# eniac/flamingo

Hardware: AMD Instinct MI355X
Metric: device-resident aggregate+unmask GB/s, N clients × L int32 per round (higher is better)
Workload: dtype u32

## Files before the change

### flamingo_amd/_lib.py

```python
from __future__ import annotations

import ctypes
import os

HERE = os.path.dirname(os.path.abspath(__file__))
LIB_PATH = os.environ.get("FLM_LIB_PATH") or os.path.join(HERE, "lib", "libflamingo_hip.so")

_u8p = ctypes.POINTER(ctypes.c_uint8)
_i8p = ctypes.POINTER(ctypes.c_int8)
_u32p = ctypes.POINTER(ctypes.c_uint32)
_i64p = ctypes.POINTER(ctypes.c_int64)
_f32p = ctypes.POINTER(ctypes.c_float)
_vp = ctypes.c_void_p
_sz = ctypes.c_size_t
_u64 = ctypes.c_uint64
_int = ctypes.c_int

SIGNATURES = {
    "flm_device_count": (_int, []),
    "flm_init": (_int, [ctypes.POINTER(_vp), _int]),
    "flm_free": (None, [_vp]),
    "flm_last_error": (ctypes.c_char_p, [_vp]),
    "flm_version": (ctypes.c_char_p, []),
    "flm_ctx_stream": (_vp, [_vp]),
# ... 32 lines not shown
    "flm_last_plan": (_int, [_vp, ctypes.POINTER(_int), ctypes.POINTER(_int), ctypes.POINTER(_int),
                             ctypes.POINTER(_int)]),
    "flm_set_tuning": (_int, [_vp, ctypes.c_char_p, _int]),
    "flm_get_tuning": (_int, [_vp, ctypes.c_char_p, ctypes.POINTER(_int)]),
    "flm_plan_aggregate": (_int, [_int, _int, _sz, _int, _int, _sz, _sz, _sz, _u64, _vp, _int,
                                  ctypes.POINTER(_int), ctypes.POINTER(_int)]),
    "flm_ec_combine": (_int, [_vp, _u8p, _u8p, _u8p, _int, _int, _int, _u8p, _u8p, _u32p]),
    "flm_ec_combine_dev": (_int, [_vp, _vp, _vp, _vp, _int, _int, _int, _vp, _vp, _vp, _vp]),
    "flm_ec_mul": (_int, [_vp, _u8p, _u8p, _int, _u8p, _u32p]),
    "flm_hash_to_curve": (_int, [_vp, _u8p, _u32p, _int, _u8p, _u32p]),
    "flm_hash_to_curve_decimal": (_int, [_vp, ctypes.c_uint32, _int, _u8p, _u32p]),
    "flm_hash_to_curve_decimal_dev": (_int, [_vp, ctypes.c_uint32, _int, _vp, _vp, _vp]),
    "flm_shamir_combine": (_int, [_vp, _u8p, _u8p, _int, _int, _u8p]),
    "flm_shamir_combine_dev": (_int, [_vp, _vp, _vp, _int, _int, _vp, _vp]),
    "flm_shamir_deal": (_int, [_vp, _u8p, _int, _int, _u32p, _int, _u8p]),
    "flm_shamir_deal_dev": (_int, [_vp, _vp, _int, _int, _vp, _int, _vp, _vp]),
    "flm_aes_gcm_xor": (_int, [_vp, _u8p, _u8p, _int, _u8p, _u8p, _sz, _int]),
    "flm_aes_gcm_xor_dev": (_int, [_vp, _vp, _vp, _int, _vp, _vp, _sz, _int, _vp]),
    "flm_aes_gcm_seal": (_int, [_vp, _u8p, _u8p, _int, _u8p, _sz, _u8p, _u8p, _sz, _u8p, _int]),
    "flm_aes_gcm_seal_dev": (_int, [_vp, _vp, _vp, _int, _vp, _sz, _vp, _vp, _sz, _vp, _int, _vp]),
    "flm_aes_gcm_open": (_int, [_vp, _u8p, _u8p, _int, _u8p, _sz, _u8p, _u8p, _u8p, _sz, _u8p, _int]),
    "flm_aes_gcm_open_dev": (_int, [_vp, _vp, _vp, _int, _vp, _sz, _vp, _vp, _vp, _sz, _vp, _int, _vp]),
    "flm_ecdsa_verify": (_int, [_vp, _u8p, _u8p, _u8p, _int, _u8p, _u32p]),
    "flm_ecdsa_verify_dev": (_int, [_vp, _vp, _vp, _vp, _int, _vp, _vp, _vp]),
    "flm_feldman_verify": (_int, [_vp, _u8p, _int, _int, _u32p, _u32p, _int, _u8p, _int, _u8p, _u8p, _u32p]),
    "flm_feldman_verify_dev": (_int, [_vp, _vp, _int, _int, _vp, _vp, _int, _vp, _int, _vp, _vp, _vp, _vp]),
    "flm_pair_units_dev": (_int, [_vp, _vp, _vp, _int, _vp, _vp, _vp, _sz, _vp, _int, _int, _vp]),
    "flm_flag_set_dev": (_int, [_vp, _vp, _vp]),
    "flm_cu_count": (_int, [_vp, _vp]),
    "flm_stream_create_cu_mask": (_int, [_vp, _vp, _int, _vp]),
    "flm_stream_destroy": (_int, [_vp, _vp]),
    "flm_shard_bounds": (_int, [_sz, _int, _int, ctypes.POINTER(_sz), ctypes.POINTER(_sz), ctypes.POINTER(_sz)]),
    "flm_client_bounds": (_int, [_int, _int, _int, ctypes.POINTER(_int), ctypes.POINTER(_int)]),
    "flm_rccl_available": (_int, []),
    "flm_comm_unique_id": (_int, [_vp]),
    "flm_comm_init_rank": (_int, [_vp, _int, _int, _vp]),
    "flm_comm_size": (_int, [_vp, ctypes.POINTER(_int), ctypes.POINTER(_int)]),
    "flm_comm_destroy": (_int, [_vp]),
    "flm_reduce_scatter_dev": (_int, [_vp, _vp, _vp, _sz, _vp]),
    "flm_all_gather_dev": (_int, [_vp, _vp, _vp, _sz, _vp]),
    "flm_group_init": (_int, [ctypes.POINTER(_vp), _int, ctypes.POINTER(_int)]),
    "flm_group_free": (None, [_vp]),
    "flm_group_last_error": (ctypes.c_char_p, [_vp]),
    "flm_group_size": (_int, [_vp]),
    "flm_group_is_loopback": (_int, [_vp]),
    "flm_group_init_flags": (_int, [ctypes.POINTER(_vp), _int, ctypes.POINTER(_int), ctypes.c_uint]),
    "flm_group_has_rccl": (_int, [_vp]),
    "flm_group_ctx": (_vp, [_vp, _int]),
    "flm_group_sync": (_int, [_vp]),
    "flm_group_aggregate_unmask": (_int, [_vp, ctypes.POINTER(_u32p), _int, _u8p, _i8p, _int, _sz, _u32p]),
    "flm_group_aggregate_unmask_dev": (_int, [_vp, ctypes.POINTER(_vp), _sz, ctypes.POINTER(_int),
                                              ctypes.POINTER(_vp), ctypes.POINTER(_vp), _int, _sz,
                                              ctypes.POINTER(_vp)]),
    "flm_store_create": (_int, [ctypes.POINTER(_vp), _vp, _vp, _sz, _int]),
    "flm_store_free": (None, [_vp]),
    "flm_store_last_error": (ctypes.c_char_p, [_vp]),
    "flm_store_count": (_int, [_vp]),
    "flm_store_add": (_int, [_vp, ctypes.c_int64, _vp, _sz]),
    "flm_store_partial": (_int, [_vp]),
    "flm_store_partial_wait": (_int, [_vp, ctypes.POINTER(ctypes.c_float)]),
    "flm_store_partial_host": (_int, [_vp, _u32p]),
    "flm_store_unmask": (_int, [_vp, _u8p, _i8p, _int, _u32p]),
    "flm_store_unmask_f32": (_int, [_vp, _u8p, _i8p, _int, _int, ctypes.c_int64, _f32p]),
    "flm_store_unmask_unpack_f32": (_int, [_vp, _u8p, _i8p, _int, _sz, _int, ctypes.c_float, _int, ctypes.c_int64, _f32p]),
    "flm_store_unmask_unpack_noise_f32": (_int, [_vp, _u8p, _i8p, _int, _sz, _int, ctypes.c_float, _int, _int,
                                                 ctypes.c_int64, _f32p]),
# ... 49 lines not shown
```

### flamingo_amd/csrc/flm_comm.hip

```cpp
#include <hip/hip_runtime.h>
#include <rccl/rccl.h>

#include <dlfcn.h>

#include <algorithm>
#include <cstdarg>
#include <cstdio>
#include <cstdlib>
#include <cstring>
#include <mutex>
#include <string>
#include <thread>
#include <vector>

#include "../../include/flamingo_hip.h"
#include "flm_internal.h"

namespace {

struct Rccl {
    void *h = nullptr;
    std::string err;
    ncclResult_t (*GetUniqueId)(ncclUniqueId *) = nullptr;
    ncclResult_t (*CommInitRank)(ncclComm_t *, int, ncclUniqueId, int) = nullptr;
// ... 119 lines not shown
        if (!c) continue;
        (void)hipSetDevice(flm::rt::device_of(ctxs[q]));
        if (c->comm && r) (void)r->CommDestroy(c->comm);
        delete c;
        *flm::rt::comm_slot(ctxs[q]) = nullptr;
    }
}
}

namespace {
constexpr uint64_t kShardAlign = 1024;

uint64_t padded_len(uint64_t L, int G) {
    const uint64_t q = kShardAlign * (uint64_t)G;
    return (L + q - 1) / q * q;
}
}

extern "C" {

int flm_shard_bounds(size_t L, int n_ranks, int rank, size_t *lo, size_t *hi, size_t *shard_words) {
    if (n_ranks < 1 || rank < 0 || rank >= n_ranks || !lo || !hi) return FLM_EINVAL;
    const uint64_t S = padded_len(L, n_ranks) / n_ranks;
    *lo = (size_t)std::min<uint64_t>((uint64_t)rank * S, L);
    *hi = (size_t)std::min<uint64_t>((uint64_t)(rank + 1) * S, L);
    if (shard_words) *shard_words = (size_t)S;
    return 0;
}

int flm_client_bounds(int N, int n_ranks, int rank, int *c0, int *c1) {
    if (N < 0 || n_ranks < 1 || rank < 0 || rank >= n_ranks || !c0 || !c1) return FLM_EINVAL;
    *c0 = (int)((int64_t)N * rank / n_ranks);
    *c1 = (int)((int64_t)N * (rank + 1) / n_ranks);
    return 0;
}

int flm_rccl_available(void) {
    Rccl *r = rccl();
    if (!r) {
        flm::rt::set_error(nullptr, FLM_EHIP, rccl_state().err.c_str());
        return 0;
    }
    return 1;
}

int flm_comm_unique_id(uint8_t id_out[128]) {
    static_assert(sizeof(ncclUniqueId) == 128, "ncclUniqueId must be 128 bytes");
    if (!id_out) return FLM_EINVAL;
    Rccl *r = rccl();
    if (!r) return flm::rt::set_error(nullptr, FLM_EHIP, "RCCL unavailable");
    ncclUniqueId id;
    ncclResult_t e = r->GetUniqueId(&id);
    if (e != ncclSuccess) return flm::rt::set_error(nullptr, FLM_EHIP, r->GetErrorString(e));
    std::memcpy(id_out, &id, sizeof id);
    return 0;
}

int flm_comm_init_rank(flm_ctx *ctx, int n_ranks, int rank, const uint8_t id[128]) {
    if (!ctx) return flm::rt::set_error(nullptr, FLM_EINVAL, "ctx is NULL");
    if (n_ranks < 1 || rank < 0 || rank >= n_ranks || !id) return fail_ctx(ctx, FLM_EINVAL, "bad rank %d of %d", rank, n_ranks);
    Rccl *r = rccl();
    if (!r) return rccl_missing(ctx);
    flm::comm_release(ctx);
    flm::rt::DeviceScope dev_scope_;
    FLM_HIPC(ctx, dev_scope_.set(flm::rt::device_of(ctx)));
    ncclUniqueId uid;
// ... 54 lines not shown

}

struct flm_group {
    int n = 0;
    std::vector<int> dev;
    std::vector<flm_ctx *> ctx;
    bool loopback = false;
    bool clique = false;
    struct Rank {
        uint32_t *partial = nullptr, *shard = nullptr;
        size_t cap_partial = 0, cap_shard = 0;
        hipEvent_t done = nullptr;
        hipEvent_t xdone = nullptr;
        bool xpending = false;
        size_t dirty = 0;
    };
    std::vector<Rank> rk;
    uint32_t *hout = nullptr;
    size_t hout_cap = 0;
    std::string err;
};

namespace {

int gfail(flm_group *g, int code, const std::string &msg) {
    if (g) g->err = msg;
    flm::rt::set_error(nullptr, code, msg.c_str());
    return code;
}

bool sharded(const flm_group *g) { return g->n > 1 || g->clique; }

int grow(flm_group *g, int r, uint32_t *&p, size_t &cap, size_t words) {
    if (words <= cap) return 0;
    (void)hipSetDevice(g->dev[r]);
    if (p) (void)hipFree(p);
    p = nullptr;
    cap = 0;
    hipError_t e = hipMalloc(&p, std::max<size_t>(words, 64) * sizeof(uint32_t));
    if (e == hipSuccess)
        e = hipMemsetAsync(p, 0, std::max<size_t>(words, 64) * sizeof(uint32_t), flm::rt::stream_of(g->ctx[r]));
    if (e != hipSuccess) return gfail(g, FLM_ENOMEM, std::string("group buffer: ") + hipGetErrorString(e));
    cap = words;
    return 0;
}

int rank_error(flm_group *g, int r, int rc) {
    return gfail(g, rc, "rank " + std::to_string(r) + ": " + flm_last_error(g->ctx[r]));
}

int exchange(flm_group *g, uint64_t S, const std::vector<uint32_t *> &shards) {
    const int G = g->n;
    if (g->loopback) {
        std::vector<const uint32_t *> parts(G);
        for (int r = 0; r < G; ++r) parts[r] = g->rk[r].partial;
        for (int r = 0; r < G; ++r) {
            hipStream_t s = flm::rt::stream_of(g->ctx[r]);
            for (int q = 0; q < G; ++q)
                if (q != r && hipStreamWaitEvent(s, g->rk[q].done, 0) != hipSuccess)
                    return gfail(g, FLM_EHIP, "hipStreamWaitEvent");
            hipError_t e = flm::launch_shard_sum(parts.data(), G, (uint64_t)r * S, S, shards[r], s);
            if (e != hipSuccess) return gfail(g, FLM_EHIP, std::string("shard_sum: ") + hipGetErrorString(e));
            if (hipEventRecord(g->rk[r].xdone, s) != hipSuccess) return gfail(g, FLM_EHIP, "hipEventRecord");
            g->rk[r].xpending = true;
        }
// ... 144 lines not shown
    return 0;
}

int flm_group_aggregate_unmask(flm_group *g, const uint32_t *const *rows, int N, const uint8_t *seeds,
                               const int8_t *signs, int K, size_t L, uint32_t *out) {
    flm::rt::DeviceScope dev_scope_;
    if (!g) return gfail(nullptr, FLM_EINVAL, "group is NULL");
    if (N < 0 || K < 0) return gfail(g, FLM_EINVAL, "negative N or K");
    if (L == 0) return 0;
    if (!out || (N > 0 && !rows) || (K > 0 && (!seeds || !signs))) return gfail(g, FLM_EINVAL, "NULL argument");
    int rc_ = 0;
    const int G = g->n;
    const bool X = sharded(g);
    const uint64_t Lp = padded_len(L, G), S = Lp / G;
    for (int r = 0; r < G; ++r) {
        if (X && (rc_ = grow(g, r, g->rk[r].partial, g->rk[r].cap_partial, Lp))) return rc_;
        if ((rc_ = grow(g, r, g->rk[r].shard, g->rk[r].cap_shard, S))) return rc_;
    }
    for (int r = 0; r < G; ++r)
        if ((rc_ = wait_previous_exchange(g, r))) return rc_;
    for (int r = 0; X && r < G; ++r)
        if ((rc_ = clear_stale_tail(g, r, L))) return rc_;
    if (g->hout_cap < L) {
        if (g->hout) (void)hipHostFree(g->hout);
        g->hout = nullptr;
        g->hout_cap = 0;
        if (hipHostMalloc(&g->hout, L * sizeof(uint32_t), hipHostMallocPortable) != hipSuccess)
            return gfail(g, FLM_ENOMEM, "group: pinned output buffer");
        g->hout_cap = L;
    }
    std::vector<int> rcs(G, 0);
    auto work = [&](int r) {
        int c0, c1;
        size_t lo, hi;
        flm_client_bounds(N, G, r, &c0, &c1);
        flm_shard_bounds(L, G, r, &lo, &hi, nullptr);
        rcs[r] = flm::rt::host_round_async(g->ctx[r], rows ? rows + c0 : nullptr, c1 - c0, seeds, signs, K, L, lo, hi,
                                           X ? g->rk[r].partial : g->rk[r].shard);
        if (!rcs[r] && hipEventRecord(g->rk[r].done, flm::rt::stream_of(g->ctx[r])) != hipSuccess) rcs[r] = FLM_EHIP;
    };
    if (G == 1) {
        work(0);
    } else {
        std::vector<std::thread> th;
        for (int r = 0; r < G; ++r) th.emplace_back(work, r);
        for (auto &t : th) t.join();
    }
    for (int r = 0; r < G; ++r)
        if (rcs[r]) return rank_error(g, r, rcs[r]);
    std::vector<uint32_t *> shards(G);
    for (int r = 0; r < G; ++r) shards[r] = g->rk[r].shard;
    if (X && (rc_ = exchange(g, S, shards))) return rc_;
    for (int r = 0; r < G; ++r) {
        size_t lo, hi;
        flm_shard_bounds(L, G, r, &lo, &hi, nullptr);
        if (hi <= lo) continue;
        (void)hipSetDevice(g->dev[r]);
        hipError_t e = hipMemcpyAsync(g->hout + lo, g->rk[r].shard, (hi - lo) * sizeof(uint32_t),
                                      hipMemcpyDeviceToHost, flm::rt::stream_of(g->ctx[r]));
        if (e != hipSuccess) return gfail(g, FLM_EHIP, std::string("shard D2H: ") + hipGetErrorString(e));
    }
    if (int rc = flm_group_sync(g)) return rc;
    flm::rt::host_copy(g->ctx[0], out, g->hout, L * sizeof(uint32_t));
    return 0;
}

int flm_group_aggregate_unmask_dev(flm_group *g, const uint32_t *const *d_rows, size_t row_pitch, const int *n_rows,
                                   const uint8_t *const *d_seeds, const int8_t *const *d_signs, int K, size_t L,
                                   uint32_t *const *d_shards) {
    flm::rt::DeviceScope dev_scope_;
    if (!g) return gfail(nullptr, FLM_EINVAL, "group is NULL");
    if (!n_rows || !d_shards || (K > 0 && (!d_seeds || !d_signs))) return gfail(g, FLM_EINVAL, "NULL argument");
    if (L == 0) return 0;
    const int G = g->n;
    const bool X = sharded(g);
    const uint64_t Lp = padded_len(L, G), S = Lp / G;
    for (int r = 0; X && r < G; ++r)
        if (int rc = grow(g, r, g->rk[r].partial, g->rk[r].cap_partial, Lp)) return rc;
    for (int r = 0; r < G; ++r)
        if (int rc = wait_previous_exchange(g, r)) return rc;
    for (int r = 0; X && r < G; ++r)
        if (int rc = clear_stale_tail(g, r, L)) return rc;
    for (int r = 0; r < G; ++r) {
        size_t lo, hi;
        flm_shard_bounds(L, G, r, &lo, &hi, nullptr);
        flm_ctx *c = g->ctx[r];
        int rc = flm_aggregate_unmask_dev(c, d_rows ? d_rows[r] : nullptr, row_pitch, n_rows[r],
                                          K ? d_seeds[r] : nullptr, K ? d_signs[r] : nullptr, K, L, lo, hi, 0,
                                          X ? g->rk[r].partial : d_shards[r], flm::rt::stream_of(c));
        if (rc) return rank_error(g, r, rc);
        if (hipEventRecord(g->rk[r].done, flm::rt::stream_of(c)) != hipSuccess) return gfail(g, FLM_EHIP, "event");
    }
    if (!X) return 0;
    return exchange(g, S, std::vector<uint32_t *>(d_shards, d_shards + G));
}

}
```

### flamingo_amd/csrc/flm_runtime.hip

```cpp
#include <hip/hip_runtime.h>
#include <hip/hip_ext.h>

#include <algorithm>
#include <cassert>
#include <cmath>
#include <cstdarg>
#include <cstdio>
#include <cstdlib>
#include <cstring>
#include <initializer_list>
#include <map>
#include <string>
#include <tuple>
#include <vector>

#include "../../include/flamingo_hip.h"
#include "flm_call_args.h"
#include "flm_copy_pool.h"
#include "flm_internal.h"
#include "flm_planner.h"

using flm::Item;
using flm::SeedRec;
using flm::plan::PlanShape;
// ... 132 lines not shown

struct flm_ctx {
    int device = 0;
    hipStream_t stream = nullptr;
    std::string err;
    DevBuf rows, out, seeds, signs, bytes_in, bytes_out;
    std::vector<SeedTable *> tables;
    SeedTable *cur_table = nullptr;
    SeedTable *pub_table = nullptr;
    DevBuf small_meta;
    bool last_small = false;
    uint64_t table_clock = 0;
    std::vector<StageSlot *> slots;
    uint64_t slot_clock = 0;
    DevBuf ec_in, ec_base, ec_scal, ec_jac, ec_out, ec_dig, ec_flags;
    void *stage[2] = {nullptr, nullptr};
    size_t stage_cap = 0;
    hipEvent_t stage_done[2] = {nullptr, nullptr};
    hipStream_t copy[4] = {nullptr, nullptr, nullptr, nullptr};
    hipEvent_t copy_done[4] = {nullptr, nullptr, nullptr, nullptr};
    hipEvent_t copy_start = nullptr;
    std::map<PlanKey, Plan *> plans;
    uint64_t plan_clock = 0;
    int last_items = 0, last_tile = 0, last_atomics = 0, last_variant = 0;
    int table_k = -1;
    int tune_variant = -1;
    int tune_subtiles = 0;
    int tune_min_items = flm::plan::kDefaultMinItems;
    int tune_ec_threads = 64;
    int tune_ec_waves = 1;
    int tune_ec_spread = 0;
    int tune_ec_terms = 1;
    int tune_ec_coop = -1;
    int tune_small = 1;
    int tune_pairing = 1;
    int tune_expand_waves = 128;
    int n_cus = 0;
    void *bounce = nullptr;
    void *bounce_dev = nullptr;
    size_t bounce_cap = 0;
    CopyPool copies;
    void *comm = nullptr;
};

namespace {

int fail(flm_ctx *ctx, int code, const char *fmt, ...) {
    char buf[512];
    va_list ap;
    va_start(ap, fmt);
    vsnprintf(buf, sizeof buf, fmt, ap);
    va_end(ap);
    if (ctx) ctx->err = buf;
    g_last_error = buf;
    return code;
}

#define FLM_ON_DEVICE(ctx)                 \
    flm::rt::DeviceScope dev_scope_;       \
    FLM_HIP((ctx), dev_scope_.set((ctx)->device))

#define FLM_HIP(ctx, expr)                                                                            \
    do {                                                                                              \
        hipError_t e_ = (expr);                                                                       \
        if (e_ != hipSuccess)                                                                         \
            return fail((ctx), FLM_EHIP, "%s failed: %s (%s:%d)", #expr, hipGetErrorString(e_), __FILE__, \
// ... 19 lines not shown
int check_noise_codec(flm_ctx *ctx, int frac_bits, float clip, int pack, int noise_bits, int64_t n, uint64_t L_params,
                      uint32_t *bias, uint32_t *bias_n) {
    bool range = false;
    const char *why = flm::rt::noise_codec_error(frac_bits, clip, pack, noise_bits, n, L_params, &range, bias, bias_n);
    return refuse(ctx, why, range ? FLM_ERANGE : FLM_EINVAL);
}
int check_aggregate_args(flm_ctx *ctx, const uint32_t *d_rows, size_t row_pitch, int N, int K, size_t L, size_t mask_lo,
                         size_t mask_hi, uint64_t prg_slot0, const uint32_t *d_out) {
    bool range = false;
    const char *why = flm::rt::aggregate_error(d_rows, row_pitch, N, K, L, mask_lo, mask_hi, prg_slot0, d_out, &range);
    return refuse(ctx, why, range ? FLM_ERANGE : FLM_EINVAL);
}

struct TuneKey {
    const char *name;
    int flm_ctx::*member;
    bool (*accepts)(int);
    const char *refusal;
};
template <int Lo, int Hi> bool within(int v) { return v >= Lo && v <= Hi; }
template <int... V> bool one_of(int v) { return ((v == V) || ...); }
const TuneKey kTuneKeys[] = {
    {"variant", &flm_ctx::tune_variant, within<-1, flm::kVarCount - 1>, "variant %d out of range"},
    {"pairing", &flm_ctx::tune_pairing, within<0, 2>, "pairing must be 0, 1 or 2"},
    {"subtiles", &flm_ctx::tune_subtiles, one_of<0, 1, 4, 16>, "subtiles must be 0 (auto), 1, 4 or 16"},
    {"ec_waves", &flm_ctx::tune_ec_waves, one_of<1, 4, 8>, "ec_waves must be 1, 4 or 8"},
    {"small", &flm_ctx::tune_small, within<0, 2>, "small must be 0 (never), 1 (auto) or 2 (when legal)"},
    {"min_items", &flm_ctx::tune_min_items, within<64, 1 << 20>, "min_items must be in [64, 2^20]"},
    {"ec_spread", &flm_ctx::tune_ec_spread, within<0, 64>, "ec_spread must be in [0, 64] KiB"},
    {"ec_terms", &flm_ctx::tune_ec_terms, one_of<1, 2, 4>, "ec_terms must be 1, 2 or 4"},
    {"ec_coop", &flm_ctx::tune_ec_coop, within<-1, 2>, "ec_coop must be -1, 0, 1 or 2"},
    {"expand_waves", &flm_ctx::tune_expand_waves, within<1, 256>, "expand_waves must be in [1, 256]"},
    {"ec_threads", &flm_ctx::tune_ec_threads, one_of<64, 128, 256>, "ec_threads must be 64, 128 or 256"},
};
const TuneKey *tune_key(const char *key) {
    for (const TuneKey &t : kTuneKeys)
        if (!std::strcmp(key, t.name)) return &t;
    return nullptr;
}

void set_last_plan(flm_ctx *ctx, int items, int tile_slots, int atomics, int variant) {
    ctx->last_items = items, ctx->last_tile = tile_slots, ctx->last_atomics = atomics, ctx->last_variant = variant;
}

StageSlot *stage_acquire(flm_ctx *ctx, size_t bytes, int *rc) {
    StageSlot *best = nullptr, *free_small = nullptr, *oldest = nullptr;
    for (StageSlot *s : ctx->slots) {
        if (s->busy && event_done(s->done)) s->busy = false;
        if (s->busy) {
            if (!oldest || s->last < oldest->last) oldest = s;
        } else if (s->cap >= bytes) {
            if (!best || s->cap < best->cap) best = s;
        } else if (!free_small) {
            free_small = s;
        }
    }
    if (!best) {
        if (ctx->slots.size() < kStageSlots) {
            best = new StageSlot();
            if (hipEventCreateWithFlags(&best->done, hipEventDisableTiming) != hipSuccess) {
                delete best;
                *rc = fail(ctx, FLM_EHIP, "staging slot: hipEventCreate failed");
                return nullptr;
            }
            ctx->slots.push_back(best);
        } else if (free_small) {
// ... 1666 lines not shown
```

### flamingo_amd/dist_recon.py

```python
from __future__ import annotations

import torch
import torch.distributed as dist

from .distributed import padded_length, shard_bounds


def pair_chunk(D: int, world: int, rank: int):
    Dc = (D + world - 1) // world if D else 0
    a = min(rank * Dc, D)
    return a, min(a + Dc, D), Dc


class ShardedReconstruction:

    def __init__(self, engine, L: int, group=None, device=None, comm: str | None = None, ec_cus: int = 0,
                 cu_pick: str = "first", force_collective: bool = False, ec_coop: int = 1):
        self.eng = engine
        self.group = group
        self.world = dist.get_world_size(group) if dist.is_initialized() else 1
        self.rank = dist.get_rank(group) if dist.is_initialized() else 0
        self.force_collective = bool(force_collective)
        if self.force_collective and not dist.is_initialized():
            raise RuntimeError("force_collective needs an initialised torch.distributed group")
        self.L = L
        self.Lp = padded_length(L, self.world)
        self.S = self.Lp // self.world
        self.lo, self.hi = shard_bounds(L, self.world, self.rank)
        self.device = torch.device("cuda", torch.cuda.current_device()) if device is None else torch.device(device)
        if comm is None:
            comm = "rccl" if ((self.world > 1 or self.force_collective) and engine.has_comm()
                              and engine.comm_size() == (self.world, self.rank)) else "torch"
        self.comm = comm
        self.ec_cus = int(ec_cus)
        self.ec_coop = int(ec_coop)
        self.pass_stream = None
        if self.ec_cus > 0:
            from .reconstruct import pick_cus
# ... 61 lines not shown
            self.eng.reduce_scatter_dev(part, out, self.S, stream=stream)
        else:
            with torch.cuda.stream(stream):
                if dist.get_backend(self.group) == "gloo":
                    host = torch.empty(self.S, dtype=part.dtype)
                    dist.reduce_scatter_tensor(host, part.cpu(), op=dist.ReduceOp.SUM, group=self.group)
                    out[: self.S].copy_(host)
                else:
                    dist.reduce_scatter_tensor(out[: self.S], part, op=dist.ReduceOp.SUM, group=self.group)

    def run(self, rows, lambdas, mi_shares, c1_mine, pair_shares_mine, pair_signs, D: int, out, stream=None):
        eng = self.eng
        main = torch.cuda.current_stream(self.device) if stream is None else stream
        M = mi_shares.shape[1]
        _, _, Dc = pair_chunk(D, self.world, self.rank)
        Dr = c1_mine.shape[0] if c1_mine is not None else 0
        with torch.cuda.stream(main):
            m_seeds = self._buf("m_seeds", (M, 32), torch.uint8)
            neg = self._buf("neg", (M,), torch.int8, -1)
            chunk = self._buf("chunk", (max(Dc, 1), 32), torch.uint8, 0)
            gathered = self._buf("gathered", (max(Dc, 1) * self.world, 32), torch.uint8)
            flags = self._buf("flags", (max(Dr, 1),), torch.int32)
            part = self._buf("part", (1, self.Lp), torch.int32, 0)
            part2 = self._buf("part2", (self.Lp,), torch.int32, 0)
        ready = torch.cuda.Event()
        ready.record(main)
        if Dr:
            self.side.wait_event(ready)
            self._ec_combine(c1_mine, pair_shares_mine, lambdas, chunk[:Dr], flags)
        done = torch.cuda.Event()
        done.record(self.side)
        ps = self._pass_begin(ready, main)
        eng.shamir_combine_dev(mi_shares, lambdas, m_seeds, stream=ps)
        eng.aggregate_unmask_dev(rows, m_seeds, neg, part[0], L=self.L, mask_lo=self.lo, mask_hi=self.hi,
                                 stream=ps)
        self._pass_end(ps, main)
        if D:
            main.wait_event(done)
            self._all_gather(chunk, gathered, main)
            eng.aggregate_unmask_dev(part, gathered[:D], pair_signs, part2, L=self.L, mask_lo=self.lo,
                                     mask_hi=self.hi, stream=main)
            src = part2
        else:
            src = part[0]
        self._reduce_scatter(src, out, main)
        return out, flags

    def report(self, rows, S_out, stream=None):
        main = torch.cuda.current_stream(self.device) if stream is None else stream
        with torch.cuda.stream(main):
            part = self._buf("report_part", (self.Lp,), torch.int32, 0)
        if rows is not None and rows.shape[0]:
            self.eng.aggregate_unmask_dev(rows, None, None, part, L=self.L, stream=main)
        else:
            with torch.cuda.stream(main):
                part[: self.L].zero_()
        self._reduce_scatter(part, S_out, main)
        return S_out

    def run_from_partial(self, S_shard, lambdas, mi_shares, c1_mine, pair_shares_mine, pair_signs, D: int, out,
                         stream=None):
        eng = self.eng
        main = torch.cuda.current_stream(self.device) if stream is None else stream
        M = mi_shares.shape[1]
        _, _, Dc = pair_chunk(D, self.world, self.rank)
        Dr = c1_mine.shape[0] if c1_mine is not None else 0
        n = self.hi - self.lo
        with torch.cuda.stream(main):
            m_seeds = self._buf("m_seeds", (M, 32), torch.uint8)
            neg = self._buf("neg", (M,), torch.int8, -1)
            chunk = self._buf("chunk", (max(Dc, 1), 32), torch.uint8, 0)
            gathered = self._buf("gathered", (max(Dc, 1) * self.world, 32), torch.uint8)
            flags = self._buf("flags", (max(Dr, 1),), torch.int32)
            part = self._buf("fp_part", (1, self.S), torch.int32, 0)
        ready = torch.cuda.Event()
        ready.record(main)
        if Dr:
# ... 17 lines not shown
```

### flamingo_amd/distributed.py

```python
from __future__ import annotations

import torch
import torch.distributed as dist

SHARD_ALIGN = 1024


def padded_length(L: int, world: int) -> int:
    q = SHARD_ALIGN * world
    return (L + q - 1) // q * q


def shard_bounds(L: int, world: int, rank: int):
    S = padded_length(L, world) // world
    lo = min(rank * S, L)
    hi = min((rank + 1) * S, L)
    return lo, hi


def client_bounds(N: int, world: int, rank: int):
    return N * rank // world, N * (rank + 1) // world


def init_rccl(engine, group=None):
    from .engine import comm_unique_id, rccl_available
    world = dist.get_world_size(group)
    rank = dist.get_rank(group)
    src = dist.get_global_rank(group, 0) if group is not None else 0
    ok, why = rccl_available()
    oks = [None] * world
    dist.all_gather_object(oks, (ok, why), group=group)
    bad = [f"rank {r}: {w}" for r, (o, w) in enumerate(oks) if not o]
    if bad:
        raise RuntimeError("RCCL unavailable on " + "; ".join(bad))
    box = [None]
    if rank == 0:
        try:
            box = [(comm_unique_id(), "")]
        except Exception as e:
            box = [(None, f"{type(e).__name__}: {e}")]
    dist.broadcast_object_list(box, src=src, group=group)
    uid, err = box[0]
    if uid is None:
        raise RuntimeError(f"RCCL unique id on rank 0 failed: {err}")
    err = ""
    try:
        engine.comm_init(world, rank, uid)
    except Exception as e:
        err = f"{type(e).__name__}: {e}"
    errs = [None] * world
    dist.all_gather_object(errs, err, group=group)
    bad = [f"rank {r}: {e}" for r, e in enumerate(errs) if e]
    if bad:
        raise RuntimeError("flm_comm_init_rank failed on " + "; ".join(bad))
# ... 29 lines not shown

class ShardedRound:

    def __init__(self, engine, L: int, group=None, device=None, buffers: int = 1, comm: str | None = None,
                 force_collective: bool = False):
        self.engine = engine
        self.group = group
        self.world = dist.get_world_size(group) if dist.is_initialized() else 1
        self.rank = dist.get_rank(group) if dist.is_initialized() else 0
        self.force_collective = bool(force_collective)
        if self.force_collective and not dist.is_initialized():
            raise RuntimeError("force_collective needs an initialised torch.distributed group")
        self._solo = self.world == 1 and not self.force_collective
        self.L = L
        self.Lp = padded_length(L, self.world)
        self.S = self.Lp // self.world
        self.lo, self.hi = shard_bounds(L, self.world, self.rank)
        dev = device if device is not None else torch.device("cuda", torch.cuda.current_device())
        if buffers not in (1, 2):
            raise ValueError("buffers must be 1 or 2")
        if comm is None:
            comm = "rccl" if (engine is not None and not self._solo and engine.has_comm()
                              and engine.comm_size() == (self.world, self.rank)) else "torch"
        if comm not in ("rccl", "torch"):
            raise ValueError("comm must be 'rccl' or 'torch'")
        if comm == "rccl" and (not engine.has_comm() or engine.comm_size() != (self.world, self.rank)):
            raise RuntimeError("comm='rccl' needs init_rccl(engine, group) first")
        self.comm = comm
        self._partials = [torch.zeros(self.Lp, dtype=torch.int32, device=dev) for _ in range(buffers)]
        self._outs = [torch.empty(self.S, dtype=torch.int32, device=dev) for _ in range(buffers)]
        self._pending = [None] * buffers
        self._comm_stream = torch.cuda.Stream(device=dev) if (comm == "rccl" and buffers == 2) else None
        self._k = 0
        self.partial, self.out = self._partials[0], self._outs[0]

    def prepare_seeds(self, d_seeds, d_signs, stream=None):
        self.K = d_seeds.shape[0]
        self.engine.seed_table_dev(d_seeds, d_signs, stream=stream)

    def compute(self, d_rows, stream=None):
        self.engine.aggregate_dev(d_rows, self.K, self.partial, L=self.L, mask_lo=self.lo, mask_hi=self.hi,
                                  stream=stream)

    def _torch_exchange(self, async_op: bool = False):
        if self.partial.is_cuda and dist.get_backend(self.group) == "gloo":
            cpu_out = torch.empty(self.out.shape, dtype=self.out.dtype)
            dist.reduce_scatter_tensor(cpu_out, self.partial.cpu(), op=dist.ReduceOp.SUM, group=self.group)
            self.out.copy_(cpu_out)
            return None
        return dist.reduce_scatter_tensor(self.out, self.partial, op=dist.ReduceOp.SUM, group=self.group,
                                          async_op=async_op)

    def exchange(self, stream=None):
        if self._solo:
            return self.partial[: self.L]
        if self.comm == "rccl":
            self.engine.reduce_scatter_dev(self.partial, self.out, self.S, stream=stream)
        else:
            st = _torch_stream(stream)
            if st is not None and self.partial.is_cuda:
                with torch.cuda.stream(st):
                    self._torch_exchange()
            else:
                self._torch_exchange()
        return self.out[: self.hi - self.lo]

    def step(self, d_rows, d_seeds, d_signs, stream=None):
        self.prepare_seeds(d_seeds, d_signs, stream)
        self.compute(d_rows, stream)
        return self.exchange(stream)

    def _async_ok(self):
        if self._solo:
            return False
        if self.comm == "rccl":
# ... 48 lines not shown
```

### flamingo_amd/engine.py

```python
from __future__ import annotations

import ctypes

import numpy as np

from . import _lib
from ._lib import p_f32, p_i8, p_i64, p_u8, p_u32

NONCE = b"\x00" * 8


def _seeds_array(seeds) -> np.ndarray:
    if isinstance(seeds, (list, tuple)):
        if len(seeds) == 0:
            return np.zeros((0, 32), np.uint8)
        if isinstance(seeds[0], (bytes, bytearray)):
            if any(len(s) != 32 for s in seeds):
                raise RuntimeError("every seed must be 32 bytes")
            return np.frombuffer(b"".join(bytes(s) for s in seeds), dtype=np.uint8).reshape(-1, 32).copy()
    a = np.ascontiguousarray(seeds, dtype=np.uint8)
    if a.size % 32:
        raise RuntimeError("seeds must be K x 32 bytes")
    return a.reshape(-1, 32)

# ... 971 lines not shown

def rccl_available():
    lib = _lib.load()
    if lib.flm_rccl_available():
        return True, ""
    return False, lib.flm_last_error(None).decode()


def comm_unique_id() -> bytes:
    lib = _lib.load()
    buf = (ctypes.c_uint8 * 128)()
    rc = lib.flm_comm_unique_id(buf)
    if rc != 0:
        raise RuntimeError(f"flm_comm_unique_id: {lib.flm_last_error(None).decode()}")
    return bytes(buf)


def shard_bounds(L: int, n_ranks: int, rank: int):
    lib = _lib.load()
    lo, hi, S = ctypes.c_size_t(), ctypes.c_size_t(), ctypes.c_size_t()
    if lib.flm_shard_bounds(int(L), int(n_ranks), int(rank), ctypes.byref(lo), ctypes.byref(hi), ctypes.byref(S)):
        raise RuntimeError("flm_shard_bounds: bad arguments")
    return lo.value, hi.value, S.value


def client_bounds(N: int, n_ranks: int, rank: int):
    lib = _lib.load()
    c0, c1 = ctypes.c_int(), ctypes.c_int()
    if lib.flm_client_bounds(int(N), int(n_ranks), int(rank), ctypes.byref(c0), ctypes.byref(c1)):
        raise RuntimeError("flm_client_bounds: bad arguments")
    return c0.value, c1.value


class DeviceGroup:

    def __init__(self, devices, force_rccl: bool = False):
        self.lib = _lib.load()
        if isinstance(devices, int):
            devices = list(range(devices))
        devices = [int(d) for d in devices]
        arr = (ctypes.c_int * len(devices))(*devices)
        g = ctypes.c_void_p()
        rc = self.lib.flm_group_init_flags(ctypes.byref(g), len(devices), arr, 1 if force_rccl else 0)
        if rc != 0:
            raise RuntimeError(f"flm_group_init({devices}): {self.lib.flm_group_last_error(None).decode()}")
        self.g = g
        self.devices = devices
        self.n = len(devices)
        self.loopback = bool(self.lib.flm_group_is_loopback(g))
        self.rccl = bool(self.lib.flm_group_has_rccl(g))
        self.force_rccl = bool(force_rccl)
        self._stores = 0
        self.retired = False
        self.engines = [MaskEngine(d, _ctx=self.lib.flm_group_ctx(g, r)) for r, d in enumerate(devices)]

    def close(self):
        if getattr(self, "g", None) is not None and self.g.value:
            if self._stores:
                raise RuntimeError(f"DeviceGroup.close: {self._stores} VectorStore(s) still use this group")
            for e in self.engines:
                e.close()
            self.lib.flm_group_free(self.g)
            self.g = None

    def __del__(self):
        try:
# ... 80 lines not shown
```

### include/flamingo_hip.h

```cpp
#ifndef FLAMINGO_HIP_H
#define FLAMINGO_HIP_H

#include <stddef.h>
#include <stdint.h>

#ifdef __cplusplus
extern "C" {
#endif

#define FLM_OK 0
#define FLM_EINVAL (-1)
#define FLM_EHIP (-2)
#define FLM_ENOMEM (-3)
#define FLM_ERANGE (-4)

typedef struct flm_ctx flm_ctx;

int flm_device_count(void);
int flm_init(flm_ctx **out, int device);
void flm_free(flm_ctx *ctx);
const char *flm_last_error(const flm_ctx *ctx);
void *flm_ctx_stream(flm_ctx *ctx);
const char *flm_version(void);

// ... 114 lines not shown
int flm_aes_gcm_seal_dev(flm_ctx *ctx, const uint8_t *d_keys, const uint8_t *d_nonces, int nonce_len,
                         const uint8_t *d_aad, size_t aad_len, const uint8_t *d_in, uint8_t *d_out, size_t len,
                         uint8_t *d_tags_out, int n, void *stream);
int flm_aes_gcm_open(flm_ctx *ctx, const uint8_t *keys, const uint8_t *nonces, int nonce_len, const uint8_t *aad,
                     size_t aad_len, const uint8_t *in, const uint8_t *tags, uint8_t *out, size_t len,
                     uint8_t *ok_out, int n);
int flm_aes_gcm_open_dev(flm_ctx *ctx, const uint8_t *d_keys, const uint8_t *d_nonces, int nonce_len,
                         const uint8_t *d_aad, size_t aad_len, const uint8_t *d_in, const uint8_t *d_tags,
                         uint8_t *d_out, size_t len, uint8_t *d_ok_out, int n, void *stream);
int flm_ecdsa_verify(flm_ctx *ctx, const uint8_t *pubkeys, const uint8_t *digests, const uint8_t *sigs, int n,
                     uint8_t *ok_out, uint32_t *flags_out);
int flm_ecdsa_verify_dev(flm_ctx *ctx, const uint8_t *d_pubkeys, const uint8_t *d_digests, const uint8_t *d_sigs,
                         int n, uint8_t *d_ok_out, uint32_t *d_flags, void *stream);
int flm_feldman_verify(flm_ctx *ctx, const uint8_t *commitments, int T, int M, const uint32_t *dealer,
                       const uint32_t *xs, int x_bits, const uint8_t *shares, int n, uint8_t *ok_out,
                       uint8_t *points_out, uint32_t *flags_out);
int flm_feldman_verify_dev(flm_ctx *ctx, const uint8_t *d_commitments, int T, int M, const uint32_t *d_dealer,
                           const uint32_t *d_xs, int x_bits, const uint8_t *d_shares, int n, uint8_t *d_ok_out,
                           uint8_t *d_points_out, uint32_t *d_flags, void *stream);
int flm_ec_mul(flm_ctx *ctx, const uint8_t *points, const uint8_t *scalars, int n, uint8_t *out, uint32_t *flags_out);
int flm_hash_to_curve(flm_ctx *ctx, const uint8_t *msgs, const uint32_t *lens, int n, uint8_t *out,
                      uint32_t *flags_out);
int flm_hash_to_curve_decimal(flm_ctx *ctx, uint32_t v0, int n, uint8_t *out, uint32_t *flags_out);
int flm_hash_to_curve_decimal_dev(flm_ctx *ctx, uint32_t v0, int n, uint8_t *d_out, uint32_t *d_flags, void *stream);


int flm_cu_count(flm_ctx *ctx, int *n_cus);
int flm_stream_create_cu_mask(flm_ctx *ctx, const uint32_t *mask, int n_words, void **stream_out);
int flm_stream_destroy(flm_ctx *ctx, void *stream);


int flm_shard_bounds(size_t L, int n_ranks, int rank, size_t *lo, size_t *hi, size_t *shard_words);
int flm_client_bounds(int N, int n_ranks, int rank, int *c0, int *c1);

int flm_rccl_available(void);
int flm_comm_destroy(flm_ctx *ctx);
int flm_comm_unique_id(uint8_t id_out[128]);
int flm_comm_init_rank(flm_ctx *ctx, int n_ranks, int rank, const uint8_t id[128]);
int flm_comm_size(flm_ctx *ctx, int *n_ranks, int *rank);
int flm_reduce_scatter_dev(flm_ctx *ctx, const uint32_t *d_send, uint32_t *d_recv, size_t recv_words, void *stream);
int flm_all_gather_dev(flm_ctx *ctx, const void *d_send, void *d_recv, size_t send_bytes, void *stream);

typedef struct flm_group flm_group;
#define FLM_GROUP_RCCL 1u
int flm_group_init(flm_group **out, int n, const int *devices);
int flm_group_init_flags(flm_group **out, int n, const int *devices, unsigned flags);
int flm_group_has_rccl(const flm_group *g);
void flm_group_free(flm_group *g);
const char *flm_group_last_error(const flm_group *g);
int flm_group_size(const flm_group *g);
int flm_group_is_loopback(const flm_group *g);
flm_ctx *flm_group_ctx(flm_group *g, int rank);
int flm_group_sync(flm_group *g);
int flm_group_aggregate_unmask(flm_group *g, const uint32_t *const *rows, int N, const uint8_t *seeds,
                               const int8_t *signs, int K, size_t L, uint32_t *out);
int flm_group_aggregate_unmask_dev(flm_group *g, const uint32_t *const *d_rows, size_t row_pitch, const int *n_rows,
                                   const uint8_t *const *d_seeds, const int8_t *const *d_signs, int K, size_t L,
                                   uint32_t *const *d_shards);


typedef struct flm_store flm_store;
int flm_store_create(flm_store **out, flm_ctx *ctx, flm_group *g, size_t L, int capacity);
void flm_store_free(flm_store *st);
const char *flm_store_last_error(const flm_store *st);
int flm_store_count(const flm_store *st);
int flm_store_add(flm_store *st, int64_t sender, const uint32_t *row, size_t n);
// ... 23 lines not shown
```

Baseline: 3260.

## Shard mask seeds across ranks instead of mask slots by default

Adds a rank_shard tuning key, default 1, under which each rank expands the full-length PRG mask for only its slice of seeds, instead of expanding every seed over only its own slot range. The sums still combine through the existing reduce-scatter. This changes how the mask-expansion work is split across devices and removes the all-gather of pairwise seeds in the recon path. The trade-off is that each rank now produces full-length partials, and the scheme relies on the reduce-scatter summing them correctly.

```diff
diff --git a/flamingo_amd/_lib.py b/flamingo_amd/_lib.py
--- a/flamingo_amd/_lib.py
+++ b/flamingo_amd/_lib.py
@@ -88,6 +88,7 @@
     "flm_stream_destroy": (_int, [_vp, _vp]),
     "flm_shard_bounds": (_int, [_sz, _int, _int, ctypes.POINTER(_sz), ctypes.POINTER(_sz), ctypes.POINTER(_sz)]),
     "flm_client_bounds": (_int, [_int, _int, _int, ctypes.POINTER(_int), ctypes.POINTER(_int)]),
+    "flm_seed_bounds": (_int, [_int, _int, _int, ctypes.POINTER(_int), ctypes.POINTER(_int)]),
     "flm_rccl_available": (_int, []),
     "flm_comm_unique_id": (_int, [_vp]),
     "flm_comm_init_rank": (_int, [_vp, _int, _int, _vp]),
diff --git a/flamingo_amd/csrc/flm_comm.hip b/flamingo_amd/csrc/flm_comm.hip
--- a/flamingo_amd/csrc/flm_comm.hip
+++ b/flamingo_amd/csrc/flm_comm.hip
@@ -175,6 +175,13 @@
     if (N < 0 || n_ranks < 1 || rank < 0 || rank >= n_ranks || !c0 || !c1) return FLM_EINVAL;
     *c0 = (int)((int64_t)N * rank / n_ranks);
     *c1 = (int)((int64_t)N * (rank + 1) / n_ranks);
+    return 0;
+}
+
+int flm_seed_bounds(int K, int n_ranks, int rank, int *k0, int *k1) {
+    if (K < 0 || n_ranks < 1 || rank < 0 || rank >= n_ranks || !k0 || !k1) return FLM_EINVAL;
+    *k0 = (int)((int64_t)K * rank / n_ranks);
+    *k1 = (int)((int64_t)K * (rank + 1) / n_ranks);
     return 0;
 }
 
@@ -295,6 +302,21 @@
 
 bool sharded(const flm_group *g) { return g->n > 1 || g->clique; }
 
+struct RankMasks {
+    int k0, k1;
+    size_t lo, hi;
+};
+RankMasks rank_masks(flm_group *g, int r, int K, size_t L) {
+    RankMasks m{0, K, 0, L};
+    int by_seeds = 1;
+    (void)flm_get_tuning(g->ctx[0], "rank_shard", &by_seeds);
+    if (by_seeds)
+        flm_seed_bounds(K, g->n, r, &m.k0, &m.k1);
+    else
+        flm_shard_bounds(L, g->n, r, &m.lo, &m.hi, nullptr);
+    return m;
+}
+
 int grow(flm_group *g, int r, uint32_t *&p, size_t &cap, size_t words) {
     if (words <= cap) return 0;
     (void)hipSetDevice(g->dev[r]);
@@ -505,11 +527,11 @@
     std::vector<int> rcs(G, 0);
     auto work = [&](int r) {
         int c0, c1;
-        size_t lo, hi;
         flm_client_bounds(N, G, r, &c0, &c1);
-        flm_shard_bounds(L, G, r, &lo, &hi, nullptr);
-        rcs[r] = flm::rt::host_round_async(g->ctx[r], rows ? rows + c0 : nullptr, c1 - c0, seeds, signs, K, L, lo, hi,
-                                           X ? g->rk[r].partial : g->rk[r].shard);
+        const RankMasks m = rank_masks(g, r, K, L);
+        rcs[r] = flm::rt::host_round_async(g->ctx[r], rows ? rows + c0 : nullptr, c1 - c0,
+                                           K ? seeds + 32 * (size_t)m.k0 : nullptr, K ? signs + m.k0 : nullptr,
+                                           m.k1 - m.k0, L, m.lo, m.hi, X ? g->rk[r].partial : g->rk[r].shard);
         if (!rcs[r] && hipEventRecord(g->rk[r].done, flm::rt::stream_of(g->ctx[r])) != hipSuccess) rcs[r] = FLM_EHIP;
     };
     if (G == 1) {
@@ -555,12 +577,12 @@
     for (int r = 0; X && r < G; ++r)
         if (int rc = clear_stale_tail(g, r, L)) return rc;
     for (int r = 0; r < G; ++r) {
-        size_t lo, hi;
-        flm_shard_bounds(L, G, r, &lo, &hi, nullptr);
+        const RankMasks m = rank_masks(g, r, K, L);
         flm_ctx *c = g->ctx[r];
         int rc = flm_aggregate_unmask_dev(c, d_rows ? d_rows[r] : nullptr, row_pitch, n_rows[r],
-                                          K ? d_seeds[r] : nullptr, K ? d_signs[r] : nullptr, K, L, lo, hi, 0,
-                                          X ? g->rk[r].partial : d_shards[r], flm::rt::stream_of(c));
+                                          K ? d_seeds[r] + 32 * (size_t)m.k0 : nullptr, K ? d_signs[r] + m.k0 : nullptr,
+                                          m.k1 - m.k0, L, m.lo, m.hi, 0, X ? g->rk[r].partial : d_shards[r],
+                                          flm::rt::stream_of(c));
         if (rc) return rank_error(g, r, rc);
         if (hipEventRecord(g->rk[r].done, flm::rt::stream_of(c)) != hipSuccess) return gfail(g, FLM_EHIP, "event");
     }
diff --git a/flamingo_amd/csrc/flm_runtime.hip b/flamingo_amd/csrc/flm_runtime.hip
--- a/flamingo_amd/csrc/flm_runtime.hip
+++ b/flamingo_amd/csrc/flm_runtime.hip
@@ -188,6 +188,7 @@
     int tune_ec_spread = 0;
     int tune_ec_terms = 1;
     int tune_ec_coop = -1;
+    int tune_rank_shard = 1;
     int tune_small = 1;
     int tune_pairing = 1;
     int tune_expand_waves = 128;
@@ -273,6 +274,7 @@
     {"ec_coop", &flm_ctx::tune_ec_coop, within<-1, 2>, "ec_coop must be -1, 0, 1 or 2"},
     {"expand_waves", &flm_ctx::tune_expand_waves, within<1, 256>, "expand_waves must be in [1, 256]"},
     {"ec_threads", &flm_ctx::tune_ec_threads, one_of<64, 128, 256>, "ec_threads must be 64, 128 or 256"},
+    {"rank_shard", &flm_ctx::tune_rank_shard, within<0, 1>, "rank_shard must be 0 (slots) or 1 (seeds)"},
 };
 const TuneKey *tune_key(const char *key) {
     for (const TuneKey &t : kTuneKeys)
diff --git a/flamingo_amd/dist_recon.py b/flamingo_amd/dist_recon.py
--- a/flamingo_amd/dist_recon.py
+++ b/flamingo_amd/dist_recon.py
@@ -3,7 +3,7 @@
 import torch
 import torch.distributed as dist
 
-from .distributed import padded_length, shard_bounds
+from .distributed import padded_length, seed_bounds, shard_bounds
 
 
 def pair_chunk(D: int, world: int, rank: int):
@@ -131,17 +131,26 @@
         done.record(self.side)
         ps = self._pass_begin(ready, main)
         eng.shamir_combine_dev(mi_shares, lambdas, m_seeds, stream=ps)
-        eng.aggregate_unmask_dev(rows, m_seeds, neg, part[0], L=self.L, mask_lo=self.lo, mask_hi=self.hi,
-                                 stream=ps)
-        self._pass_end(ps, main)
-        if D:
-            main.wait_event(done)
-            self._all_gather(chunk, gathered, main)
-            eng.aggregate_unmask_dev(part, gathered[:D], pair_signs, part2, L=self.L, mask_lo=self.lo,
-                                     mask_hi=self.hi, stream=main)
-            src = part2
-        else:
-            src = part[0]
+        src = part[0]
+        if eng.get_tuning("rank_shard"):
+            m0, m1 = seed_bounds(M, self.world, self.rank)
+            eng.aggregate_unmask_dev(rows, m_seeds[m0:m1], neg[m0:m1], part[0], L=self.L, stream=ps)
+            self._pass_end(ps, main)
+            if Dr:
+                a = pair_chunk(D, self.world, self.rank)[0]
+                main.wait_event(done)
+                eng.aggregate_unmask_dev(part, chunk[:Dr], pair_signs[a:a + Dr], part2, L=self.L, stream=main)
+                src = part2
+        else:
+            eng.aggregate_unmask_dev(rows, m_seeds, neg, part[0], L=self.L, mask_lo=self.lo, mask_hi=self.hi,
+                                     stream=ps)
+            self._pass_end(ps, main)
+            if D:
+                main.wait_event(done)
+                self._all_gather(chunk, gathered, main)
+                eng.aggregate_unmask_dev(part, gathered[:D], pair_signs, part2, L=self.L, mask_lo=self.lo,
+                                         mask_hi=self.hi, stream=main)
+                src = part2
         self._reduce_scatter(src, out, main)
         return out, flags
 
diff --git a/flamingo_amd/distributed.py b/flamingo_amd/distributed.py
--- a/flamingo_amd/distributed.py
+++ b/flamingo_amd/distributed.py
@@ -20,6 +20,14 @@
 
 def client_bounds(N: int, world: int, rank: int):
     return N * rank // world, N * (rank + 1) // world
+
+
+def seed_bounds(K: int, world: int, rank: int):
+    return K * rank // world, K * (rank + 1) // world
+
+
+def seed_slice(K: int, lo: int, hi: int, Lp: int):
+    return K * lo // Lp, K * hi // Lp
 
 
 def init_rccl(engine, group=None):
@@ -115,15 +123,33 @@
         self._pending = [None] * buffers
         self._comm_stream = torch.cuda.Stream(device=dev) if (comm == "rccl" and buffers == 2) else None
         self._k = 0
+        self._mask = None
         self.partial, self.out = self._partials[0], self._outs[0]
 
+    def seed_range(self, K: int):
+        lo, hi = self.lo, self.hi
+        if (lo, hi) == shard_bounds(self.L, self.world, self.rank):
+            lo, hi = self.rank * self.S, (self.rank + 1) * self.S
+        elif hi >= self.L:
+            hi = self.Lp
+        return seed_slice(K, lo, hi, self.Lp)
+
     def prepare_seeds(self, d_seeds, d_signs, stream=None):
-        self.K = d_seeds.shape[0]
+        K = d_seeds.shape[0]
+        if self.engine.get_tuning("rank_shard"):
+            k0, k1 = self.seed_range(K)
+            self._mask = (0, self.L)
+        else:
+            k0, k1 = 0, K
+            self._mask = (self.lo, self.hi)
+        self.K = k1 - k0
+        if self.K != K:
+            d_seeds, d_signs = d_seeds[k0:k1], d_signs[k0:k1]
         self.engine.seed_table_dev(d_seeds, d_signs, stream=stream)
 
     def compute(self, d_rows, stream=None):
-        self.engine.aggregate_dev(d_rows, self.K, self.partial, L=self.L, mask_lo=self.lo, mask_hi=self.hi,
-                                  stream=stream)
+        lo, hi = self._mask or (self.lo, self.hi)
+        self.engine.aggregate_dev(d_rows, self.K, self.partial, L=self.L, mask_lo=lo, mask_hi=hi, stream=stream)
 
     def _torch_exchange(self, async_op: bool = False):
         if self.partial.is_cuda and dist.get_backend(self.group) == "gloo":
diff --git a/flamingo_amd/engine.py b/flamingo_amd/engine.py
--- a/flamingo_amd/engine.py
+++ b/flamingo_amd/engine.py
@@ -1027,6 +1027,14 @@
     return c0.value, c1.value
 
 
+def seed_bounds(K: int, n_ranks: int, rank: int):
+    lib = _lib.load()
+    k0, k1 = ctypes.c_int(), ctypes.c_int()
+    if lib.flm_seed_bounds(int(K), int(n_ranks), int(rank), ctypes.byref(k0), ctypes.byref(k1)):
+        raise RuntimeError("flm_seed_bounds: bad arguments")
+    return k0.value, k1.value
+
+
 class DeviceGroup:
 
     def __init__(self, devices, force_rccl: bool = False):
diff --git a/include/flamingo_hip.h b/include/flamingo_hip.h
--- a/include/flamingo_hip.h
+++ b/include/flamingo_hip.h
@@ -170,6 +170,7 @@
 
 int flm_shard_bounds(size_t L, int n_ranks, int rank, size_t *lo, size_t *hi, size_t *shard_words);
 int flm_client_bounds(int N, int n_ranks, int rank, int *c0, int *c1);
+int flm_seed_bounds(int K, int n_ranks, int rank, int *k0, int *k1);
 
 int flm_rccl_available(void);
 int flm_comm_destroy(flm_ctx *ctx);
```

Result: no change. 3260 (-0.0%).
